# Factral/unsupervised-hyperspectral-nerf

Measured on AMD Instinct MI355X. Metric: train rays/sec (hotdog-shaped 31-band, C2), higher is better.
Workload: dtype f32; 1 GPU; C2 hotdog 31-band rgb+spectral train step (fwd+loss+bwd+Adam); rays_per_gpu=4096, samples_per_ray=64, bands=31, endmembers=6, global_rays=4096, hash_table=16x2^19x2 f32, parallelism=dp1

## Files before the change

### unsupervised-hyperspectral-nerf_amd/csrc/umhs_hashgrid.hip

```cpp
#include <atomic>
#include <cstdlib>

#include "umhs_hashgrid_part.h"

__global__ __launch_bounds__(256) void hashgrid_fwd_kernel(const float* __restrict__ pos01,
                                                           const float2* __restrict__ table,
                                                           const float* __restrict__ scalings, int64_t n, int n_levels,
                                                           int log2_T, float* __restrict__ enc, int64_t stride_n,
                                                           int64_t stride_l) {
  int64_t i = (int64_t)blockIdx.x * 256 + threadIdx.x;
  if (i >= n) return;
  const float px = pos01[3 * i], py = pos01[3 * i + 1], pz = pos01[3 * i + 2];
  const int l = (int)blockIdx.y;
  HashCorners h = hash_corners(px, py, pz, scalings[l], (1u << log2_T) - 1u, (uint32_t)l << log2_T);
  float2 f[8];
  hash_gather8(table, h, f);
  const float2 r = hash_trilerp(f, h.ox, h.oy, h.oz);
  float* o = enc + i * stride_n + (int64_t)l * stride_l;
  if (((stride_n | stride_l) & 1) == 0) {
    *reinterpret_cast<float2*>(o) = r;
  } else {
    o[0] = r.x, o[1] = r.y;
  }
}

extern "C" int umhs_hashgrid_fwd(const float* pos01, const float* table, const float* scalings, int64_t n,
                                 int n_levels, int log2_T, float* enc, int64_t stride_n, int64_t stride_l,
                                 umhs_stream_t stream) {
  if (n < 0 || !table || !scalings) return UMHS_ERR_ARG;
  if (n_levels < 1 || n_levels > 32 || log2_T < 1 || log2_T > 24) return UMHS_ERR_UNSUPPORTED;
  if (n == 0) return UMHS_OK;
  if (!pos01 || !enc) return UMHS_ERR_ARG;
  if (((uintptr_t)table & 15) || ((uintptr_t)enc & 7)) return UMHS_ERR_ARG;
  const float2* t2 = reinterpret_cast<const float2*>(table);
  dim3 grid((unsigned)((n + 255) / 256), (unsigned)n_levels);
  hipLaunchKernelGGL(hashgrid_fwd_kernel, grid, dim3(256), 0, umhs_s(stream), pos01, t2, scalings, n, n_levels, log2_T, enc, stride_n, stride_l);
  UMHS_CHECK_LAUNCH();
  return UMHS_OK;
}

__global__ __launch_bounds__(256) void hashgrid_bwd_kernel(const float* __restrict__ pos01,
                                                           const float* __restrict__ d_enc, int64_t stride_n,
                                                           int64_t stride_l, const float* __restrict__ scalings,
                                                           int64_t n, int log2_T, float* __restrict__ d_table, int level0) {
  int64_t i = (int64_t)blockIdx.x * 256 + threadIdx.x;
  if (i >= n) return;
  int l = level0 + blockIdx.y;
  const float* g = d_enc + i * stride_n + (int64_t)l * stride_l;
  float g0 = g[0], g1 = g[1];
  if (g0 == 0.0f && g1 == 0.0f) return;
  HashCorners h = hash_corners(pos01[3 * i], pos01[3 * i + 1], pos01[3 * i + 2], scalings[l],
                               (1u << log2_T) - 1u, (uint32_t)l << log2_T);
  float ox = h.ox, oy = h.oy, oz = h.oz, rx = 1.0f - ox, ry = 1.0f - oy, rz = 1.0f - oz;
  float w[8];
  w[0] = ox * oy * oz, w[3] = rx * oy * oz, w[1] = ox * ry * oz, w[2] = rx * ry * oz;
  w[4] = ox * oy * rz, w[7] = rx * oy * rz, w[5] = ox * ry * rz, w[6] = rx * ry * rz;
#pragma unroll
  for (int c = 0; c < 8; ++c) {
    if (w[c] != 0.0f) {
      atomicAdd(d_table + 2 * (size_t)h.idx[c], w[c] * g0);
      atomicAdd(d_table + 2 * (size_t)h.idx[c] + 1, w[c] * g1);
    }
  }
}

static_assert(HB_RUN == 512, "hashgrid_fwd_count_kernel's workgroup is one run of the partition");
__global__ __launch_bounds__(HB_RUN) void hashgrid_fwd_count_kernel(const float2* __restrict__ table, float* __restrict__ enc, int64_t stride_n,
                                                                 int64_t stride_l, HbArgs a) {
  __shared__ uint32_t cursor[HB_MAX_NB];
  const int tid = threadIdx.x, lane = tid & 63, wg = blockIdx.x, l = blockIdx.y;
  if (tid < HB_MAX_NB) cursor[tid] = 0;
  __syncthreads();
  const int64_t i = (int64_t)wg * HB_RUN + tid;
  const bool act = i < a.n;
  const int64_t ii = act ? i : a.n - 1;
  const uint32_t mask = (1u << a.log2_T) - 1u, base = (uint32_t)l << a.log2_T;
  const HashCorners h = hash_corners(a.pos01[3 * ii], a.pos01[3 * ii + 1], a.pos01[3 * ii + 2], a.scalings[l], mask, base);
  HashGather hg;
  hash_gather8_issue(table, h, hg);
  __builtin_amdgcn_sched_barrier(0);
  uint32_t slot[8];
#pragma unroll
  for (int c = 0; c < 8; ++c) slot[c] = h.idx[c] - base;
  const uint32_t kx = act ? h.fx : 0xffffffffu, ky = act ? h.fy : 0u, kz = act ? h.fz : 0u;
  const uint32_t kf = act ? (h.eqx | (h.eqy << 1) | (h.eqz << 2)) : (0x80000000u | (uint32_t)lane);
  hb_count_sample(slot, kx, ky, kz, kf, act, a.bucket_bits, lane, cursor);
  __syncthreads();
  if (tid < a.nb) a.wg_counts[((size_t)l * a.nwg + wg) * a.nb + tid] = cursor[tid];
  __builtin_amdgcn_sched_barrier(0);
  float2 f[8];
  hash_gather8_select(h, hg, f);
  const float2 r = hash_trilerp(f, h.ox, h.oy, h.oz);
  if (act) {
    float* o = enc + i * stride_n + (int64_t)l * stride_l;
    if (((stride_n | stride_l) & 1) == 0) {
      *reinterpret_cast<float2*>(o) = r;
    } else {
      o[0] = r.x, o[1] = r.y;
    }
  }
}

static inline int hb_scatter_wgs(int n_levels) {
  static const int forced = [] {
    const char* e = getenv("UMHS_HB_WGS");
    return e ? atoi(e) : 0;
  }();
  int w = forced > 0 ? forced : 1024 / (n_levels > 0 ? n_levels : 1);
  w = (w + 7) / 8 * 8;
  return w < 8 ? 8 : w;
}

struct HbLayout {
  int bucket_bits, nb, nwg;
  size_t cap;
  size_t counts, offsets, lmax, wg_counts, wg_prefix, recs, total;
};

static HbLayout hb_layout(int64_t n, int n_levels, int log2_T) {
  HbLayout w{};
  if (n <= 0 || n_levels < 1 || log2_T < 2) return w;
  w.bucket_bits = log2_T < HB_BUCKET_BITS ? log2_T : HB_BUCKET_BITS, w.nb = 1 << (log2_T - w.bucket_bits);
  if (w.nb > HB_MAX_NB) return w;
  w.nwg = (int)((n + HB_RUN - 1) / HB_RUN);
  w.cap = ((size_t)n * HB_CAP_PER_SAMPLE + 7) & ~(size_t)7;
  if (w.cap >= ((size_t)1 << 28)) return w;
  const auto align = [](size_t x) { return (x + 255) & ~(size_t)255; };
  const size_t m = (size_t)n_levels * w.nb, wg_bytes = align((size_t)n_levels * w.nwg * w.nb * 4);
  w.counts = 0, w.offsets = m * 4, w.lmax = 2 * m * 4;
  w.wg_counts = align((2 * m + (size_t)n_levels * HB_LMAX_PARTS) * 4);
  w.wg_prefix = w.wg_counts + wg_bytes;
  w.recs = w.wg_prefix + wg_bytes;
  w.total = 256 + w.recs + align((size_t)n_levels * w.cap * 16);
  return w;
}

extern "C" size_t umhs_hashgrid_bwd_workspace_bytes(int64_t n, int n_levels, int log2_T) { return hb_layout(n, n_levels, log2_T).total; }

static int hb_args(HbArgs* a, const float* pos01, const float* scalings, int64_t n, int ws_begin, int ws_levels, int log2_T,
                   void* workspace, size_t workspace_bytes) {
  const HbLayout w = hb_layout(n, ws_levels, log2_T);
  if (w.total == 0) return UMHS_ERR_UNSUPPORTED;
  if (!workspace || workspace_bytes < w.total) return UMHS_ERR_WORKSPACE;
  a->pos01 = pos01, a->d_enc = nullptr, a->sn = 0, a->sl = 0, a->scalings = scalings, a->n = n;
  a->log2_T = log2_T, a->bucket_bits = w.bucket_bits, a->nb = w.nb, a->level0 = ws_begin;
  a->nlev = ws_levels, a->lev_off = 0, a->overwrite = 0, a->grad_mask = 0;
  a->adam = HbAdam{};
  a->nwg = w.nwg, a->cap = (uint32_t)w.cap;
  char* const base = reinterpret_cast<char*>(((uintptr_t)workspace + 255) & ~(uintptr_t)255);
  a->counts = reinterpret_cast<uint32_t*>(base + w.counts), a->offsets = reinterpret_cast<uint32_t*>(base + w.offsets);
  a->lmax = reinterpret_cast<uint32_t*>(base + w.lmax);
  a->wg_counts = reinterpret_cast<uint32_t*>(base + w.wg_counts), a->wg_prefix = reinterpret_cast<uint32_t*>(base + w.wg_prefix);
  a->recs = reinterpret_cast<uint4*>(base + w.recs);
  return UMHS_OK;
}

static int hb_run_prepare(const HbArgs& a, int n_levels, int count_wgs, umhs_stream_t stream) {
  if (a.grad_mask && !a.d_enc) return UMHS_ERR_ARG;
  if (n_levels != a.nlev) return UMHS_ERR_ARG;
  dim3 pgrid((unsigned)(count_wgs > 0 && count_wgs < a.nwg ? count_wgs : a.nwg), (unsigned)n_levels);
  hipLaunchKernelGGL(hg_partition_kernel<false>, pgrid, dim3(256), 0, umhs_s(stream), a);
  hipLaunchKernelGGL(hg_wgscan_kernel, dim3((unsigned)a.nb, (unsigned)n_levels), dim3(256), 0, umhs_s(stream), a);
  hipLaunchKernelGGL(hg_scan_kernel, dim3((unsigned)n_levels), dim3(64), 0, umhs_s(stream), a);
  UMHS_CHECK_LAUNCH();
  return UMHS_OK;
}

static int hb_run_apply(const HbArgs& a, int n_levels, float* d_table, umhs_stream_t stream) {
  if (!a.d_enc || !d_table || !a.pos01 || !a.scalings) return UMHS_ERR_ARG;
  int per_level = hb_scatter_wgs(n_levels);
  if (per_level > HB_LMAX_PARTS) per_level = HB_LMAX_PARTS;
  if (per_level > ((a.nwg + 7) / 8) * 8) per_level = ((a.nwg + 7) / 8) * 8;
  dim3 pgrid((unsigned)per_level, (unsigned)n_levels);
  hipLaunchKernelGGL(hg_partition_kernel<true>, pgrid, dim3(256), 0, umhs_s(stream), a);
  const size_t lds = (size_t)(2 << a.bucket_bits) * 8;
  {
    static std::atomic<size_t> granted[16];
    int dev = 0;
    if (hipGetDevice(&dev) != hipSuccess || dev < 0 || dev >= 16) dev = -1;
    if (dev < 0 || granted[dev].load(std::memory_order_relaxed) < lds) {
      if (hipFuncSetAttribute(reinterpret_cast<const void*>(hg_reduce_kernel), hipFuncAttributeMaxDynamicSharedMemorySize,
                              (int)lds) != hipSuccess)
        return UMHS_ERR_LAUNCH;
      if (dev >= 0) granted[dev].store(lds, std::memory_order_relaxed);
    }
  }
  hipLaunchKernelGGL(hg_reduce_kernel, dim3((unsigned)a.nb, (unsigned)n_levels), dim3(1024), lds, umhs_s(stream), a, d_table);
  UMHS_CHECK_LAUNCH();
  return UMHS_OK;
}

extern "C" int umhs_hashgrid_bwd(const float* pos01, const float* d_enc, int64_t stride_n, int64_t stride_l,
                                 const float* scalings, int64_t n, int level_begin, int n_levels, int log2_T,
                                 float* d_table, int overwrite, void* workspace, size_t workspace_bytes,
                                 umhs_stream_t stream) {
  if (n < 0 || !scalings || !d_table || level_begin < 0) return UMHS_ERR_ARG;
  if (n > 0 && (!pos01 || !d_enc)) return UMHS_ERR_ARG;
  if (overwrite && (!workspace || n == 0)) {
    if (hipMemsetAsync(d_table + (((size_t)level_begin << log2_T) * 2), 0, ((size_t)n_levels << log2_T) * 8, umhs_s(stream)) !=
        hipSuccess)
      return UMHS_ERR_LAUNCH;
  }
  if (n_levels < 1 || level_begin + n_levels > 32 || log2_T < 2 || log2_T > 24) return UMHS_ERR_UNSUPPORTED;
  if (n == 0) return UMHS_OK;
  if (!workspace) {
    dim3 grid((unsigned)((n + 255) / 256), (unsigned)n_levels);
    hipLaunchKernelGGL(hashgrid_bwd_kernel, grid, dim3(256), 0, umhs_s(stream), pos01, d_enc, stride_n, stride_l,
                       scalings, n, log2_T, d_table, level_begin);
    UMHS_CHECK_LAUNCH();
    return UMHS_OK;
  }
  HbArgs a;
  int rc = hb_args(&a, pos01, scalings, n, level_begin, n_levels, log2_T, workspace, workspace_bytes);
  if (rc) return rc;
  if ((uintptr_t)d_table & 15) return UMHS_ERR_WORKSPACE;
  a.d_enc = d_enc, a.sn = stride_n, a.sl = stride_l, a.overwrite = overwrite, a.grad_mask = 1;
  rc = hb_run_prepare(a, n_levels, 0, stream);
  if (rc) return rc;
  return hb_run_apply(a, n_levels, d_table, stream);
}

extern "C" int umhs_hashgrid_bwd_prepare(const float* pos01, const float* scalings, int64_t n, int level_begin, int n_levels,
                                         int log2_T, void* workspace, size_t workspace_bytes, umhs_stream_t stream) {
  if (n < 0 || !scalings || level_begin < 0) return UMHS_ERR_ARG;
  if (n_levels < 1 || level_begin + n_levels > 32 || log2_T < 2 || log2_T > 24) return UMHS_ERR_UNSUPPORTED;
  if (n == 0) return UMHS_OK;
  if (!pos01) return UMHS_ERR_ARG;
  HbArgs a;
  int rc = hb_args(&a, pos01, scalings, n, level_begin, n_levels, log2_T, workspace, workspace_bytes);
  if (rc) return rc;
  const int throttle = 16;
  return hb_run_prepare(a, n_levels, throttle, stream);
}

extern "C" int umhs_hashgrid_fwd_count(const float* pos01, const float* table, const float* scalings, int64_t n, int n_levels, int log2_T,
                                       float* enc, int64_t stride_n, int64_t stride_l, void* workspace, size_t workspace_bytes,
                                       umhs_stream_t stream) {
  if (n < 0 || !table || !scalings) return UMHS_ERR_ARG;
  if (n_levels < 1 || n_levels > 32 || log2_T < 2 || log2_T > 24) return UMHS_ERR_UNSUPPORTED;
  if (n == 0) return UMHS_OK;
  if (!pos01 || !enc) return UMHS_ERR_ARG;
  if (((uintptr_t)table & 15) || ((uintptr_t)enc & 7)) return UMHS_ERR_ARG;
  HbArgs a;
  int rc = hb_args(&a, pos01, scalings, n, 0, n_levels, log2_T, workspace, workspace_bytes);
  if (rc) return rc;
  hipLaunchKernelGGL(hashgrid_fwd_count_kernel, dim3((unsigned)a.nwg, (unsigned)n_levels), dim3(HB_RUN), 0, umhs_s(stream),
                     reinterpret_cast<const float2*>(table), enc, stride_n, stride_l, a);
  UMHS_CHECK_LAUNCH();
  return UMHS_OK;
}

extern "C" int umhs_hashgrid_bwd_prepare_counted(const float* pos01, const float* scalings, int64_t n, int n_levels, int log2_T,
                                                 void* workspace, size_t workspace_bytes, umhs_stream_t stream) {
  if (n < 0 || !pos01 || !scalings) return UMHS_ERR_ARG;
  if (n_levels < 1 || n_levels > 32 || log2_T < 2 || log2_T > 24) return UMHS_ERR_UNSUPPORTED;
  if (n == 0) return UMHS_OK;
  HbArgs a;
  int rc = hb_args(&a, pos01, scalings, n, 0, n_levels, log2_T, workspace, workspace_bytes);
  if (rc) return rc;
  hipLaunchKernelGGL(hg_wgscan_kernel, dim3((unsigned)a.nb, (unsigned)n_levels), dim3(256), 0, umhs_s(stream), a);
  hipLaunchKernelGGL(hg_scan_kernel, dim3((unsigned)n_levels), dim3(64), 0, umhs_s(stream), a);
  UMHS_CHECK_LAUNCH();
  return UMHS_OK;
}

static int hb_apply(const float* pos01, const float* d_enc, int64_t stride_n, int64_t stride_l, const float* scalings, int64_t n,
                    int level_begin, int n_levels, int ws_level_begin, int ws_n_levels, int log2_T, float* d_table, int overwrite,
                    const HbAdam* adam, void* workspace, size_t workspace_bytes, umhs_stream_t stream) {
  if (n < 0 || !scalings || !d_table || level_begin < 0) return UMHS_ERR_ARG;
  if (n > 0 && (!pos01 || !d_enc)) return UMHS_ERR_ARG;
  if (n_levels < 1 || level_begin < ws_level_begin || level_begin + n_levels > ws_level_begin + ws_n_levels ||
      ws_level_begin + ws_n_levels > 32 || log2_T < 2 || log2_T > 24)
    return UMHS_ERR_UNSUPPORTED;
  if ((uintptr_t)d_table & 15) return UMHS_ERR_WORKSPACE;
  if (n == 0) {
    if (overwrite && hipMemsetAsync(d_table + (((size_t)level_begin << log2_T) * 2), 0, ((size_t)n_levels << log2_T) * 8,
                                    umhs_s(stream)) != hipSuccess)
      return UMHS_ERR_LAUNCH;
    return UMHS_OK;
  }
  HbArgs a;
  int rc = hb_args(&a, pos01, scalings, n, ws_level_begin, ws_n_levels, log2_T, workspace, workspace_bytes);
  if (rc) return rc;
  a.d_enc = d_enc, a.sn = stride_n, a.sl = stride_l, a.lev_off = level_begin - ws_level_begin, a.overwrite = overwrite;
  if (adam) a.adam = *adam;
  return hb_run_apply(a, n_levels, d_table, stream);
}

extern "C" int umhs_hashgrid_bwd_apply(const float* pos01, const float* d_enc, int64_t stride_n, int64_t stride_l,
                                       const float* scalings, int64_t n, int level_begin, int n_levels, int ws_level_begin,
                                       int ws_n_levels, int log2_T, float* d_table, int overwrite, void* workspace,
                                       size_t workspace_bytes, umhs_stream_t stream) {
  return hb_apply(pos01, d_enc, stride_n, stride_l, scalings, n, level_begin, n_levels, ws_level_begin, ws_n_levels, log2_T, d_table,
                  overwrite, nullptr, workspace, workspace_bytes, stream);
}

extern "C" int umhs_hashgrid_bwd_apply_adam(const float* pos01, const float* d_enc, int64_t stride_n, int64_t stride_l,
                                            const float* scalings, int64_t n, int level_begin, int n_levels, int ws_level_begin,
                                            int ws_n_levels, int log2_T, float* d_table, void* workspace, size_t workspace_bytes,
                                            float* table_params, float* exp_avg, float* exp_avg_sq, float lr, float beta1,
                                            float beta2, float eps, int64_t step, int adam_level_begin, umhs_stream_t stream) {
  if (!table_params || !exp_avg || !exp_avg_sq || step < 1 || adam_level_begin < 0) return UMHS_ERR_ARG;
  if (((uintptr_t)table_params | (uintptr_t)exp_avg | (uintptr_t)exp_avg_sq) & 15) return UMHS_ERR_ARG;
  if (n <= 0) return UMHS_ERR_UNSUPPORTED;
  const AdamBias bc = adam_bias(lr, beta1, beta2, step);
  HbAdam ad;
  ad.p = table_params, ad.m = exp_avg, ad.v = exp_avg_sq, ad.lr_bc1 = bc.lr_bc1, ad.b1 = beta1, ad.b2 = beta2, ad.eps = eps;
  ad.sqrt_bc2 = bc.sqrt_bc2, ad.level_begin = adam_level_begin;
  return hb_apply(pos01, d_enc, stride_n, stride_l, scalings, n, level_begin, n_levels, ws_level_begin, ws_n_levels, log2_T, d_table,
                  1, &ad, workspace, workspace_bytes, stream);
}

__global__ __launch_bounds__(256) void enc_gather_kernel(const float2* __restrict__ in, const int64_t* __restrict__ idx, int64_t m,
                                                         int64_t n, float2* __restrict__ out) {
  const int64_t i = (int64_t)blockIdx.x * 256 + threadIdx.x;
  if (i >= n) return;
  int64_t j = idx[i];
  j = j < 0 ? 0 : (j >= m ? m - 1 : j);
  const int l = blockIdx.y;
  out[(int64_t)l * n + i] = in[(int64_t)l * m + j];
}

extern "C" int umhs_enc_gather(const float* enc_in, const int64_t* index, int64_t m, int64_t n, int n_levels, float* enc_out,
                               umhs_stream_t stream) {
  if (m < 0 || n < 0 || n_levels < 1 || n_levels > 64) return UMHS_ERR_ARG;
  if (n == 0) return UMHS_OK;
  if (m < 1 || !enc_in || !index || !enc_out || (((uintptr_t)enc_in | (uintptr_t)enc_out) & 7)) return UMHS_ERR_ARG;
  hipLaunchKernelGGL(enc_gather_kernel, dim3((unsigned)((n + 255) / 256), (unsigned)n_levels), dim3(256), 0, umhs_s(stream),
                     reinterpret_cast<const float2*>(enc_in), index, m, n, reinterpret_cast<float2*>(enc_out));
  UMHS_CHECK_LAUNCH();
  return UMHS_OK;
}
```

### unsupervised-hyperspectral-nerf_amd/csrc/umhs_hashgrid_part.h

```cpp
#pragma once
#include "umhs_adam.h"
#include "umhs_hash.h"

#define HB_BUCKET_BITS 13
#define HB_MAX_NB 128
#define HB_SPT 2
#define HB_RUN (256 * HB_SPT)
#define HB_CAP_PER_SAMPLE 5
#define HB_MERGE_MIN 16
#define HB_POISON 0xffffffffu
#define HB_LMAX_PARTS 128

struct HbAdam {
  float *p, *m, *v;
  float lr_bc1, b1, b2, eps, sqrt_bc2;
  int level_begin;
};

struct HbArgs {
  HbAdam adam;
  const float* pos01;
  const float* d_enc;
  int64_t sn, sl;
  const float* scalings;
  int64_t n;
  int log2_T, bucket_bits, nb, level0, nlev;
  int lev_off;
  int grad_mask;
  uint32_t *counts, *offsets;
  uint32_t *wg_counts, *wg_prefix;
  int nwg;
  uint32_t* lmax;
  uint4* recs;
  uint32_t cap;
  int overwrite;
};

template <int D>
__device__ __forceinline__ float row_shr(float v) {
  return __int_as_float(__builtin_amdgcn_update_dpp(0, __float_as_int(v), 0x110 + D, 0xF, 0xF, true));
}
template <int D>
__device__ __forceinline__ uint32_t row_shr_u(uint32_t v) {
  return (uint32_t)__builtin_amdgcn_update_dpp(0, (int)v, 0x110 + D, 0xF, 0xF, true);
}
__device__ __forceinline__ int row_shl1(int v) {
  return __builtin_amdgcn_update_dpp(0, v, 0x101, 0xF, 0xF, true);
}
__device__ __forceinline__ uint32_t wave_scan_incl_dpp(uint32_t v) {
  v += row_shr_u<1>(v);
  v += row_shr_u<2>(v);
  v += row_shr_u<4>(v);
  v += row_shr_u<8>(v);
  v += (uint32_t)__builtin_amdgcn_update_dpp(0, (int)v, 0x142, 0xA, 0xF, false);
  v += (uint32_t)__builtin_amdgcn_update_dpp(0, (int)v, 0x143, 0xC, 0xF, false);
  return v;
}
__device__ __forceinline__ uint32_t wave_max_u32_dpp(uint32_t v) {
  v = max(v, row_shr_u<1>(v)), v = max(v, row_shr_u<2>(v)), v = max(v, row_shr_u<4>(v)), v = max(v, row_shr_u<8>(v));
  return max(max((uint32_t)__builtin_amdgcn_readlane((int)v, 15), (uint32_t)__builtin_amdgcn_readlane((int)v, 31)),
             max((uint32_t)__builtin_amdgcn_readlane((int)v, 47), (uint32_t)__builtin_amdgcn_readlane((int)v, 63)));
}
template <int D>
__device__ __forceinline__ void seg_scan_step(float2 (&val)[8], bool& f, int l16) {
  const bool take = l16 >= D && !f;
#pragma unroll
  for (int c = 0; c < 8; ++c) {
    const float px = row_shr<D>(val[c].x), py = row_shr<D>(val[c].y);
    if (take) val[c].x += px, val[c].y += py;
  }
  const int pf = (int)row_shr_u<D>((uint32_t)f);
  if (l16 >= D) f = f || pf;
}

#ifdef UMHS_HG_STAMP
__device__ unsigned long long g_hg_stamp[2][16][16];
#define HG_STAMP_DECL unsigned long long hgs_acc_[15] = {}, hgs_t_ = hg_now_(false)
__device__ __forceinline__ unsigned long long hg_now_(bool drain) {
  unsigned long long t;
  __builtin_amdgcn_sched_barrier(0);
  if (drain) {
    asm volatile("s_waitcnt vmcnt(0)\n\ts_memtime %0\n\ts_waitcnt lgkmcnt(0)" : "=s"(t)::"memory");
  } else {
    asm volatile("s_memtime %0\n\ts_waitcnt lgkmcnt(0)" : "=s"(t)::"memory");
  }
  __builtin_amdgcn_sched_barrier(0);
  return t;
}
#define HG_STAMP(k_)                              \
  do {                                            \
    const unsigned long long n_ = hg_now_(false); \
    hgs_acc_[k_] += n_ - hgs_t_, hgs_t_ = n_;     \
  } while (0)
#define HG_STAMP_DRAIN(k_)                       \
  do {                                           \
    const unsigned long long n_ = hg_now_(true); \
    hgs_acc_[k_] += n_ - hgs_t_, hgs_t_ = n_;    \
  } while (0)
#define HG_STAMP_FLUSH(kern_, lev_)                                                                                     \
  do {                                                                                                                  \
    if ((threadIdx.x & 63) == 0) {                                                                                      \
      _Pragma("unroll") for (int q_ = 0; q_ < 15; ++q_) if (hgs_acc_[q_]) atomicAdd(&g_hg_stamp[kern_][(lev_) & 15][q_], hgs_acc_[q_]); \
      atomicAdd(&g_hg_stamp[kern_][(lev_) & 15][15], 1ull);                                                             \
    }                                                                                                                   \
  } while (0)
extern "C" int umhs_debug_hg_stamps(unsigned long long* out) {
  return (int)hipMemcpyFromSymbol(out, HIP_SYMBOL(g_hg_stamp), sizeof(unsigned long long) * 2 * 16 * 16);
}
extern "C" int umhs_debug_hg_stamps_clear() {
  static unsigned long long z[2 * 16 * 16] = {};
  return (int)hipMemcpyToSymbol(HIP_SYMBOL(g_hg_stamp), z, sizeof(z));
}
#else
#define HG_STAMP_DECL \
  do {                \
  } while (0)
#define HG_STAMP(k_) \
  do {               \
  } while (0)
#define HG_STAMP_DRAIN(k_) \
  do {                     \
  } while (0)
#define HG_STAMP_FLUSH(kern_, lev_) \
  do {                              \
  } while (0)
#endif


struct HbIn {
  float g[HB_SPT][2], p[HB_SPT][3];
  uint32_t c[2], mb[2];
};

template <bool SCATTER>
__device__ __forceinline__ void hb_load(const HbArgs& a, const int wg, const int lev, const int l, HbIn& in) {
  const int tid = threadIdx.x;
#pragma unroll
  for (int k = 0; k < HB_SPT; ++k) {
    const int64_t i = (int64_t)wg * HB_RUN + k * 256 + tid, ii = i < a.n ? i : a.n - 1;
    in.g[k][0] = in.g[k][1] = 0.0f;
    if (SCATTER || a.grad_mask) {
      const float* g = a.d_enc + ii * a.sn + (int64_t)l * a.sl;
      if (((a.sn | a.sl) & 1) == 0 && (((uintptr_t)a.d_enc) & 7) == 0) {
        const float2 g2 = *reinterpret_cast<const float2*>(g);
        in.g[k][0] = g2.x, in.g[k][1] = g2.y;
      } else {
        in.g[k][0] = g[0], in.g[k][1] = g[1];
      }
    }
    in.p[k][0] = a.pos01[3 * ii], in.p[k][1] = a.pos01[3 * ii + 1], in.p[k][2] = a.pos01[3 * ii + 2];
  }
  in.c[0] = in.c[1] = in.mb[0] = in.mb[1] = 0u;
  if (SCATTER && tid < 64) {
#pragma unroll
    for (int h = 0; h < 2; ++h) {
      const int bk = tid + 64 * h;
      if (bk < a.nb) {
        const size_t o = ((size_t)lev * a.nwg + wg) * a.nb + bk;
        in.c[h] = a.wg_counts[o];
        in.mb[h] = a.offsets[lev * a.nb + bk] + a.wg_prefix[o];
      }
    }
  }
}

template <bool SCATTER>
__device__ __forceinline__ void hg_partition_body(const HbArgs& a, const int wg, const int lev, const int l, const float s, const HbIn& in,
                                                  uint32_t& wgmax) {
  __shared__ uint32_t cursor[HB_MAX_NB];
  __shared__ uint32_t delta[HB_MAX_NB];
  __shared__ uint32_t ltotal;
  constexpr int MAXREC = SCATTER ? HB_RUN * 4 : 1;
  __shared__ uint4 stage[MAXREC];
  const int tid = threadIdx.x, lane = tid & 63;
  HG_STAMP_DECL;
  if (!SCATTER && tid < HB_MAX_NB) cursor[tid] = 0;
  if (SCATTER && tid < 64) {
    uint32_t carry = 0;
#pragma unroll
    for (int h = 0; h < 2; ++h) {
      const int bk = tid + 64 * h;
      const uint32_t c = in.c[h], mb = in.mb[h];
      const uint32_t incl = wave_scan_incl_dpp(c);
      const uint32_t first = carry + incl - c;
      carry += (uint32_t)__builtin_amdgcn_readlane((int)incl, 63);
      cursor[bk] = first, delta[bk] = mb - first;
    }
    if (tid == 0) ltotal = carry;
  }
  __syncthreads();
  const uint32_t mask = (1u << a.log2_T) - 1u;
  const int bb = a.bucket_bits;
  uint4* const __restrict__ out = a.recs + (size_t)lev * a.cap;
  const bool staged = SCATTER && ltotal <= (uint32_t)MAXREC;
  if (SCATTER) HG_STAMP_DRAIN(0);
  uint32_t vmax = 0u;
  auto emit = [&](const uint32_t meta, const float vx, const float vy, const float ox) {
    const uint32_t b = __builtin_amdgcn_ubfe(meta, (uint32_t)bb, (uint32_t)(24 - bb));
    const uint32_t pos = atomicAdd(&cursor[b], 1u);
    if (!SCATTER) return;
    const uint4 r = make_uint4(__float_as_uint(vx), __float_as_uint(vy), __float_as_uint(ox), meta);
    if (staged)
      stage[pos] = r;
    else
      out[delta[b] + pos] = r;
  };
#pragma unroll
  for (int k = 0; k < HB_SPT; ++k) {
    const int64_t i = (int64_t)wg * HB_RUN + k * 256 + tid;
    bool act = false;
    float g0 = 0.0f, g1 = 0.0f, ox = 0.0f, oy = 0.0f, oz = 0.0f;
    uint32_t kx = 0xffffffffu, ky = 0, kz = 0, kf = 0x80000000u | (uint32_t)lane;
    uint32_t slot[8];
#pragma unroll
    for (int c = 0; c < 8; ++c) slot[c] = 0;
    if (SCATTER) HG_STAMP_DRAIN(1);
    if (i < a.n) {
      g0 = in.g[k][0], g1 = in.g[k][1];
      if (!a.grad_mask || g0 != 0.0f || g1 != 0.0f) {
        act = true;
        HashCorners h = hash_corners(in.p[k][0], in.p[k][1], in.p[k][2], s, mask, 0u);
        ox = h.ox, oy = h.oy, oz = h.oz;
#pragma unroll
        for (int c = 0; c < 8; ++c) slot[c] = h.idx[c];
        kx = h.fx, ky = h.fy, kz = h.fz, kf = h.eqx | (h.eqy << 1) | (h.eqz << 2);
      }
    }
    if (SCATTER) HG_STAMP(2);
    const int l16 = lane & 15;
    const uint32_t px_ = row_shr_u<1>(kx), py_ = row_shr_u<1>(ky), pz_ = row_shr_u<1>(kz), pf_ = row_shr_u<1>(kf);
    bool head = (l16 == 0) | (px_ != kx) | (py_ != ky) | (pz_ != kz) | (pf_ != kf);
    const bool merging = __builtin_popcountll(__builtin_amdgcn_ballot_w64(!head)) >= HB_MERGE_MIN;
    if (!merging) head = true;
    const int nhead = merging ? row_shl1((int)head) : 1;
    const bool tail = act && (l16 == 15 || nhead);
    const bool solo = head && tail;
    const float rx = 1.0f - ox, ry = 1.0f - oy, rz = 1.0f - oz;
    float2 val[8];
    if (SCATTER && merging) {
      float w[8];
      w[0] = ox * oy * oz, w[3] = rx * oy * oz, w[1] = ox * ry * oz, w[2] = rx * ry * oz;
      w[4] = ox * oy * rz, w[7] = rx * oy * rz, w[5] = ox * ry * rz, w[6] = rx * ry * rz;
#pragma unroll
      for (int c = 0; c < 8; ++c) val[c] = act ? make_float2(w[c] * g0, w[c] * g1) : make_float2(0.0f, 0.0f);
      bool f = head;
      seg_scan_step<1>(val, f, l16), seg_scan_step<2>(val, f, l16);
      seg_scan_step<4>(val, f, l16), seg_scan_step<8>(val, f, l16);
    }
    if (SCATTER) HG_STAMP(3);
    if (tail) {
      const uint32_t single = 15u << 24;
      if (solo) {
        const uint32_t pm = slot[HASH_FI[0]] ^ slot[HASH_CI[0]];
        const float wyz[4] = {oy * oz, ry * oz, oy * rz, ry * rz};
        if (SCATTER) vmax = max(vmax, max(__float_as_uint(fabsf(g0)), __float_as_uint(fabsf(g1))));
        if ((pm >> bb) == 0) {
          const uint32_t km = (pm ? (uint32_t)(31 - __clz((int)pm)) : 15u) << 24;
          uint32_t meta[4], pos[4], bk[4];
#pragma unroll
          for (int p = 0; p < 4; ++p) {
            meta[p] = slot[HASH_FI[p]] | km;
            bk[p] = __builtin_amdgcn_ubfe(meta[p], (uint32_t)bb, (uint32_t)(24 - bb));
            pos[p] = atomicAdd(&cursor[bk[p]], 1u);
          }
          if (SCATTER) {
#pragma unroll
            for (int p = 0; p < 4; ++p) {
              const uint4 r = make_uint4(__float_as_uint(g0 * wyz[p]), __float_as_uint(g1 * wyz[p]), __float_as_uint(ox), meta[p]);
              if (staged)
                stage[pos[p]] = r;
              else
                out[delta[bk[p]] + pos[p]] = r;
            }
          }
        } else {
#pragma unroll
          for (int p = 0; p < 4; ++p) {
            const float gx = g0 * wyz[p], gy = g1 * wyz[p];
            emit(slot[HASH_FI[p]] | single, gx * rx, gy * rx, 0.0f);
            emit(slot[HASH_CI[p]] | single, gx * ox, gy * ox, 0.0f);
          }
        }
      } else {
#pragma unroll
        for (int c = 0; c < 8; ++c) {
          if (SCATTER) vmax = max(vmax, max(__float_as_uint(fabsf(val[c].x)), __float_as_uint(fabsf(val[c].y))));
          emit(slot[c] | single, SCATTER ? val[c].x : 0.0f, SCATTER ? val[c].y : 0.0f, 0.0f);
        }
      }
    }
    if (SCATTER) HG_STAMP(4);
  }
  if (!SCATTER) {
    __syncthreads();
    if (tid < a.nb) a.wg_counts[((size_t)lev * a.nwg + wg) * a.nb + tid] = cursor[tid];
    return;
  }
  vmax = wave_max_u32_dpp(vmax);
  if (lane == 0 && vmax > 0u) atomicMax(&wgmax, vmax);
  HG_STAMP(5);
  __syncthreads();
  HG_STAMP(6);
  if (staged) {
    char* const ob = reinterpret_cast<char*>(out);
    const uint32_t total = ltotal;
    for (uint32_t i = tid; i < total; i += 256) {
      const uint4 r = stage[i];
      const uint32_t b = __builtin_amdgcn_ubfe(r.w, (uint32_t)bb, (uint32_t)(24 - bb));
      *reinterpret_cast<uint4*>(ob + (size_t)((delta[b] + i) << 4)) = r;
    }
  }
  HG_STAMP_DRAIN(7);
  HG_STAMP_FLUSH(0, l);
}

__device__ __forceinline__ void hb_count_sample(const uint32_t (&slot)[8], const uint32_t kx, const uint32_t ky, const uint32_t kz, const uint32_t kf,
                                                const bool act, const int bb, const int lane, uint32_t* __restrict__ cursor) {
  const int l16 = lane & 15;
  const uint32_t px_ = row_shr_u<1>(kx), py_ = row_shr_u<1>(ky), pz_ = row_shr_u<1>(kz), pf_ = row_shr_u<1>(kf);
  bool head = (l16 == 0) | (px_ != kx) | (py_ != ky) | (pz_ != kz) | (pf_ != kf);
  const bool merging = __builtin_popcountll(__builtin_amdgcn_ballot_w64(!head)) >= HB_MERGE_MIN;
  if (!merging) head = true;
  const int nhead = merging ? row_shl1((int)head) : 1;
  const bool tail = act && (l16 == 15 || nhead);
  const bool solo = head && tail;
  if (tail) {
    if (solo) {
      const uint32_t pm = slot[3] ^ slot[0];
      static_assert(HASH_FI[0] == 3 && HASH_FI[1] == 2 && HASH_FI[2] == 7 && HASH_FI[3] == 6 && HASH_CI[0] == 0, "corner order");
      atomicAdd(&cursor[slot[3] >> bb], 1u), atomicAdd(&cursor[slot[2] >> bb], 1u);
      atomicAdd(&cursor[slot[7] >> bb], 1u), atomicAdd(&cursor[slot[6] >> bb], 1u);
      if ((pm >> bb) != 0) {
        atomicAdd(&cursor[slot[0] >> bb], 1u), atomicAdd(&cursor[slot[1] >> bb], 1u);
        atomicAdd(&cursor[slot[4] >> bb], 1u), atomicAdd(&cursor[slot[5] >> bb], 1u);
      }
    } else {
      atomicAdd(&cursor[slot[0] >> bb], 1u), atomicAdd(&cursor[slot[1] >> bb], 1u);
      atomicAdd(&cursor[slot[2] >> bb], 1u), atomicAdd(&cursor[slot[3] >> bb], 1u);
      atomicAdd(&cursor[slot[4] >> bb], 1u), atomicAdd(&cursor[slot[5] >> bb], 1u);
      atomicAdd(&cursor[slot[6] >> bb], 1u), atomicAdd(&cursor[slot[7] >> bb], 1u);
    }
  }
}

template <bool SCATTER>
__global__ __launch_bounds__(256) void hg_partition_kernel(HbArgs a) {
  const int lev = a.lev_off + blockIdx.y, l = a.level0 + lev;
  const float s = a.scalings[l];
  __shared__ uint32_t wgmax;
  HbIn cur;
  if (threadIdx.x == 0) wgmax = 0;
  if (SCATTER) {
    const int per = (a.nwg + 7) >> 3, q = (int)(gridDim.x >> 3);
    const int x = (int)(blockIdx.x & 7u), end = min(a.nwg, (x + 1) * per);
    int wg = x * per + (int)(blockIdx.x >> 3);
    const uint32_t lmax0 = a.lmax[(size_t)lev * HB_LMAX_PARTS];
    if (wg >= end) return;
    hb_load<true>(a, wg, lev, l, cur);
    if (lmax0 == HB_POISON) return;
    while (true) {
      const int nxt = wg + q;
      HbIn nx;
      if (nxt < end) hb_load<true>(a, nxt, lev, l, nx);
      hg_partition_body<true>(a, wg, lev, l, s, cur, wgmax);
      if (nxt >= end) break;
      cur = nx, wg = nxt;
      __syncthreads();
    }
    __syncthreads();
    if (threadIdx.x == 0 && wgmax) a.lmax[(size_t)lev * HB_LMAX_PARTS + (blockIdx.x % HB_LMAX_PARTS)] = wgmax;
  } else {
    for (int wg = blockIdx.x; wg < a.nwg; wg += gridDim.x) {
      hb_load<false>(a, wg, lev, l, cur);
      hg_partition_body<false>(a, wg, lev, l, s, cur, wgmax);
      __syncthreads();
    }
  }
}

__global__ __launch_bounds__(256) void hg_wgscan_kernel(HbArgs a) {
  __shared__ uint32_t wsum[4];
  const int tid = threadIdx.x, lane = tid & 63, wv = tid >> 6, b = blockIdx.x, lev = blockIdx.y;
  const int per = (a.nwg + 255) / 256, w0 = min(a.nwg, tid * per), w1 = min(a.nwg, w0 + per);
  const uint32_t* __restrict__ col = a.wg_counts + (size_t)lev * a.nwg * a.nb + b;
  uint32_t* __restrict__ pre = a.wg_prefix + (size_t)lev * a.nwg * a.nb + b;
  uint32_t sum = 0;
  for (int w = w0; w < w1; ++w) sum += col[(size_t)w * a.nb];
  uint32_t incl = sum;
#pragma unroll
  for (int d = 1; d < 64; d <<= 1) {
    const uint32_t o = __shfl_up(incl, d, 64);
    if (lane >= d) incl += o;
  }
  if (lane == 63) wsum[wv] = incl;
  __syncthreads();
  uint32_t run = incl - sum, total = 0;
#pragma unroll
  for (int k = 0; k < 4; ++k) {
    if (k < wv) run += wsum[k];
    total += wsum[k];
  }
  for (int w = w0; w < w1; ++w) {
    pre[(size_t)w * a.nb] = run;
    run += col[(size_t)w * a.nb];
  }
  if (tid == 0) a.counts[lev * a.nb + b] = total;
}

__global__ void hg_scan_kernel(HbArgs a) {
  const int lane = threadIdx.x, lev = blockIdx.x;
  uint32_t carry = 0;
  for (int b0 = 0; b0 < a.nb; b0 += 64) {
    const int b = b0 + lane;
    const uint32_t c = b < a.nb ? a.counts[lev * a.nb + b] : 0u;
    uint32_t incl = c;
#pragma unroll
    for (int d = 1; d < 64; d <<= 1) {
      const uint32_t o = __shfl_up(incl, d, 64);
      if (lane >= d) incl += o;
    }
    if (b < a.nb) a.offsets[lev * a.nb + b] = carry + incl - c;
    carry += __shfl(incl, 63, 64);
  }
  for (int j = lane; j < HB_LMAX_PARTS; j += 64) a.lmax[(size_t)lev * HB_LMAX_PARTS + j] = (j == 0 && carry > a.cap) ? HB_POISON : 0u;
}

__device__ __forceinline__ unsigned long long hb_fixed(const float x) {
  const float fl = floorf(x);
  const int hi = (int)fl;
  const uint32_t lo = (uint32_t)((x - fl) * 4294967296.0f);
  return ((unsigned long long)(uint32_t)hi << 32) | lo;
}

__global__ __launch_bounds__(1024) void hg_reduce_kernel(HbArgs a, float* __restrict__ d_table) {
  extern __shared__ __attribute__((aligned(16))) long long tile[];
  const int tid = threadIdx.x, b = blockIdx.x, lev = a.lev_off + blockIdx.y, l = a.level0 + lev;
  HG_STAMP_DECL;
  const uint32_t start = a.offsets[lev * a.nb + b], cnt = a.counts[lev * a.nb + b];
  const int nsl = 2 << a.bucket_bits;
  const size_t slab = 2 * (((size_t)l << a.log2_T) + ((size_t)b << a.bucket_bits));
  const bool adam = a.adam.p != nullptr && l >= a.adam.level_begin;
  auto step4 = [&](const float4& g, float4& pp, float4& mm, float4& vv) {
    adam_update(pp.x, mm.x, vv.x, g.x, a.adam.lr_bc1, a.adam.b1, a.adam.b2, a.adam.eps, a.adam.sqrt_bc2);
    adam_update(pp.y, mm.y, vv.y, g.y, a.adam.lr_bc1, a.adam.b1, a.adam.b2, a.adam.eps, a.adam.sqrt_bc2);
    adam_update(pp.z, mm.z, vv.z, g.z, a.adam.lr_bc1, a.adam.b1, a.adam.b2, a.adam.eps, a.adam.sqrt_bc2);
    adam_update(pp.w, mm.w, vv.w, g.w, a.adam.lr_bc1, a.adam.b1, a.adam.b2, a.adam.eps, a.adam.sqrt_bc2);
  };
  const uint32_t lmax_bits =
      wave_max_u32_dpp(max(a.lmax[(size_t)lev * HB_LMAX_PARTS + (tid & 63)], a.lmax[(size_t)lev * HB_LMAX_PARTS + 64 + (tid & 63)]));
  const bool nan_level = lmax_bits >= 0x7f800000u && (cnt != 0 || lmax_bits == HB_POISON);
  const bool from_tile = cnt != 0 && !nan_level;
  if (!from_tile && !a.overwrite && !nan_level) return;
  int kfix = 0;
  if (from_tile) {
    for (int i = tid; i < nsl; i += 1024) tile[i] = 0;
    int e;
    (void)frexpf(__uint_as_float(lmax_bits), &e);
    const int hb = 33 - __clz(cnt);
    kfix = min(62 - hb - e, 150);
    __syncthreads();
    const uint4* __restrict__ rp = a.recs + (size_t)lev * a.cap + start;
    typedef unsigned long long u64;
    u64* ut = reinterpret_cast<u64*>(tile);
    const uint32_t lowmask = (1u << a.bucket_bits) - 1u;
    const float fscale = ldexpf(1.0f, kfix - 32);
    auto add = [&](const uint4& r) {
      const float vx = __uint_as_float(r.x), vy = __uint_as_float(r.y), ox = __uint_as_float(r.z);
      const uint32_t s = r.w & lowmask, kk = (r.w >> 24) & 15u;
      const float rx = (1.0f - ox) * fscale, oxs = ox * fscale;
      atomicAdd(&ut[2 * s], hb_fixed(vx * rx)), atomicAdd(&ut[2 * s + 1], hb_fixed(vy * rx));
      if (kk != 15u) {
        const uint32_t cs = s ^ (((2u << kk) - 1u) & lowmask);
        atomicAdd(&ut[2 * cs], hb_fixed(vx * oxs)), atomicAdd(&ut[2 * cs + 1], hb_fixed(vy * oxs));
      }
    };
    uint32_t i = tid;
    HG_STAMP(0);
    const uint32_t last = cnt - 1;
    auto load4 = [&](uint4 (&r)[4], const uint32_t at) {
#pragma unroll
      for (int u = 0; u < 4; ++u) r[u] = rp[min(at + 1024u * u, last)];
    };
    auto add4 = [&](const uint4 (&r)[4], const uint32_t at) {
      add(r[0]);
#pragma unroll
      for (int u = 1; u < 4; ++u)
        if (at + 1024u * u < cnt) add(r[u]);
    };
    uint4 ra[4], rb[4];
    if (i < cnt) {
      load4(ra, i);
      while (true) {
        HG_STAMP_DRAIN(1);
        load4(rb, i + 4096u);
        add4(ra, i);
        HG_STAMP(3);
        i += 4096u;
        if (i >= cnt) break;
        HG_STAMP_DRAIN(1);
        load4(ra, i + 4096u);
        add4(rb, i);
        HG_STAMP(3);
        i += 4096u;
        if (i >= cnt) break;
      }
    }
    HG_STAMP_DRAIN(3);
    __syncthreads();
    HG_STAMP(4);
  }
  float* const dst = d_table + slab;
  const float qnan = __uint_as_float(0x7fc00000u);
  for (int j0 = tid * 4; j0 < nsl; j0 += 4 * 4096) {
    float4 pp[4], mm[4], vv[4], dd[4];
#pragma unroll
    for (int c = 0; c < 4; ++c) {
      const int j = min(j0 + c * 4096, nsl - 4);
      if (adam) {
        pp[c] = *reinterpret_cast<const float4*>(a.adam.p + slab + j), mm[c] = *reinterpret_cast<const float4*>(a.adam.m + slab + j);
        vv[c] = *reinterpret_cast<const float4*>(a.adam.v + slab + j);
      }
      if (!a.overwrite) dd[c] = *reinterpret_cast<const float4*>(dst + j);
    }
#pragma unroll
    for (int c = 0; c < 4; ++c) {
      const int j = j0 + c * 4096;
      if (j < nsl) {
        float4 d = a.overwrite ? make_float4(0.f, 0.f, 0.f, 0.f) : dd[c];
        if (nan_level) {
          d = make_float4(qnan, qnan, qnan, qnan);
        } else if (from_tile) {
          d.x += (float)ldexp((double)tile[j], -kfix), d.y += (float)ldexp((double)tile[j + 1], -kfix);
          d.z += (float)ldexp((double)tile[j + 2], -kfix), d.w += (float)ldexp((double)tile[j + 3], -kfix);
        }
        *reinterpret_cast<float4*>(dst + j) = d;
        if (adam) {
          step4(d, pp[c], mm[c], vv[c]);
          *reinterpret_cast<float4*>(a.adam.p + slab + j) = pp[c];
          *reinterpret_cast<float4*>(a.adam.m + slab + j) = mm[c];
          *reinterpret_cast<float4*>(a.adam.v + slab + j) = vv[c];
        }
      }
    }
  }
  HG_STAMP_DRAIN(5);
  HG_STAMP_FLUSH(1, l);
}
```

Measured before the change: 6.010 million rays/s.

## Make hashgrid reduce kernel persistent with cross-tile prefetch of records and headers

Result: no change. 5.960 million rays/s (-0.8%).

```diff
diff --git a/unsupervised-hyperspectral-nerf_amd/csrc/umhs_hashgrid.hip b/unsupervised-hyperspectral-nerf_amd/csrc/umhs_hashgrid.hip
--- a/unsupervised-hyperspectral-nerf_amd/csrc/umhs_hashgrid.hip
+++ b/unsupervised-hyperspectral-nerf_amd/csrc/umhs_hashgrid.hip
@@ -174,18 +174,37 @@
   dim3 pgrid((unsigned)per_level, (unsigned)n_levels);
   hipLaunchKernelGGL(hg_partition_kernel<true>, pgrid, dim3(256), 0, umhs_s(stream), a);
   const size_t lds = (size_t)(2 << a.bucket_bits) * 8;
+  int cus = 0;
   {
     static std::atomic<size_t> granted[16];
+    static std::atomic<int> cu_count[16];
     int dev = 0;
     if (hipGetDevice(&dev) != hipSuccess || dev < 0 || dev >= 16) dev = -1;
     if (dev < 0 || granted[dev].load(std::memory_order_relaxed) < lds) {
-      if (hipFuncSetAttribute(reinterpret_cast<const void*>(hg_reduce_kernel), hipFuncAttributeMaxDynamicSharedMemorySize,
+      if (hipFuncSetAttribute(reinterpret_cast<const void*>(hg_reduce_kernel<true>), hipFuncAttributeMaxDynamicSharedMemorySize,
+                              (int)lds) != hipSuccess ||
+          hipFuncSetAttribute(reinterpret_cast<const void*>(hg_reduce_kernel<false>), hipFuncAttributeMaxDynamicSharedMemorySize,
                               (int)lds) != hipSuccess)
         return UMHS_ERR_LAUNCH;
       if (dev >= 0) granted[dev].store(lds, std::memory_order_relaxed);
     }
-  }
-  hipLaunchKernelGGL(hg_reduce_kernel, dim3((unsigned)a.nb, (unsigned)n_levels), dim3(1024), lds, umhs_s(stream), a, d_table);
+    if (dev >= 0) cus = cu_count[dev].load(std::memory_order_relaxed);
+    if (cus <= 0) {
+      int cur = dev;
+      if ((cur < 0 && hipGetDevice(&cur) != hipSuccess) || hipDeviceGetAttribute(&cus, hipDeviceAttributeMultiprocessorCount, cur) != hipSuccess ||
+          cus <= 0)
+        return UMHS_ERR_LAUNCH;
+      if (dev >= 0) cu_count[dev].store(cus, std::memory_order_relaxed);
+    }
+  }
+  const int tiles = a.nb * n_levels;
+  int wgs = cus;
+  if (const char* e = getenv("UMHS_HR_WGS"); e && *e) wgs = atoi(e) < 1 ? 1 : atoi(e);
+  if (wgs > tiles) wgs = tiles;
+  if (a.bucket_bits == HB_BUCKET_BITS)
+    hipLaunchKernelGGL(hg_reduce_kernel<true>, dim3((unsigned)wgs), dim3(1024), lds, umhs_s(stream), a, d_table, tiles);
+  else
+    hipLaunchKernelGGL(hg_reduce_kernel<false>, dim3((unsigned)wgs), dim3(1024), lds, umhs_s(stream), a, d_table, tiles);
   UMHS_CHECK_LAUNCH();
   return UMHS_OK;
 }
diff --git a/unsupervised-hyperspectral-nerf_amd/csrc/umhs_hashgrid_part.h b/unsupervised-hyperspectral-nerf_amd/csrc/umhs_hashgrid_part.h
--- a/unsupervised-hyperspectral-nerf_amd/csrc/umhs_hashgrid_part.h
+++ b/unsupervised-hyperspectral-nerf_amd/csrc/umhs_hashgrid_part.h
@@ -104,6 +104,10 @@
       atomicAdd(&g_hg_stamp[kern_][(lev_) & 15][15], 1ull);                                                             \
     }                                                                                                                   \
   } while (0)
+#define HG_STAMP_RESET                                                   \
+  do {                                                                   \
+    _Pragma("unroll") for (int q_ = 0; q_ < 15; ++q_) hgs_acc_[q_] = 0; \
+  } while (0)
 extern "C" int umhs_debug_hg_stamps(unsigned long long* out) {
   return (int)hipMemcpyFromSymbol(out, HIP_SYMBOL(g_hg_stamp), sizeof(unsigned long long) * 2 * 16 * 16);
 }
@@ -123,6 +127,9 @@
   } while (0)
 #define HG_STAMP_FLUSH(kern_, lev_) \
   do {                              \
+  } while (0)
+#define HG_STAMP_RESET \
+  do {                 \
   } while (0)
 #endif
 
@@ -432,117 +439,182 @@
   return ((unsigned long long)(uint32_t)hi << 32) | lo;
 }
 
-__global__ __launch_bounds__(1024) void hg_reduce_kernel(HbArgs a, float* __restrict__ d_table) {
+#define HG_READ4(r_) asm volatile("" ::"v"((r_)[0]), "v"((r_)[1]), "v"((r_)[2]), "v"((r_)[3]))
+typedef uint32_t hb_rec __attribute__((ext_vector_type(4)));
+template <bool FULL>
+__global__ __launch_bounds__(1024) void hg_reduce_kernel(HbArgs a, float* __restrict__ d_table, const int tiles) {
   extern __shared__ __attribute__((aligned(16))) long long tile[];
-  const int tid = threadIdx.x, b = blockIdx.x, lev = a.lev_off + blockIdx.y, l = a.level0 + lev;
+  typedef unsigned long long u64;
+  const int tid = threadIdx.x, lane = tid & 63, G = (int)gridDim.x;
+  const int nsl = FULL ? (2 << HB_BUCKET_BITS) : (2 << a.bucket_bits), nbs = a.log2_T - a.bucket_bits;
+  const uint32_t lowmask = FULL ? (1u << HB_BUCKET_BITS) - 1u : (1u << a.bucket_bits) - 1u;
+  const float qnan = __uint_as_float(0x7fc00000u);
+  u64* const ut = reinterpret_cast<u64*>(tile);
   HG_STAMP_DECL;
-  const uint32_t start = a.offsets[lev * a.nb + b], cnt = a.counts[lev * a.nb + b];
-  const int nsl = 2 << a.bucket_bits;
-  const size_t slab = 2 * (((size_t)l << a.log2_T) + ((size_t)b << a.bucket_bits));
-  const bool adam = a.adam.p != nullptr && l >= a.adam.level_begin;
   auto step4 = [&](const float4& g, float4& pp, float4& mm, float4& vv) {
     adam_update(pp.x, mm.x, vv.x, g.x, a.adam.lr_bc1, a.adam.b1, a.adam.b2, a.adam.eps, a.adam.sqrt_bc2);
     adam_update(pp.y, mm.y, vv.y, g.y, a.adam.lr_bc1, a.adam.b1, a.adam.b2, a.adam.eps, a.adam.sqrt_bc2);
     adam_update(pp.z, mm.z, vv.z, g.z, a.adam.lr_bc1, a.adam.b1, a.adam.b2, a.adam.eps, a.adam.sqrt_bc2);
     adam_update(pp.w, mm.w, vv.w, g.w, a.adam.lr_bc1, a.adam.b1, a.adam.b2, a.adam.eps, a.adam.sqrt_bc2);
   };
-  const uint32_t lmax_bits =
-      wave_max_u32_dpp(max(a.lmax[(size_t)lev * HB_LMAX_PARTS + (tid & 63)], a.lmax[(size_t)lev * HB_LMAX_PARTS + 64 + (tid & 63)]));
-  const bool nan_level = lmax_bits >= 0x7f800000u && (cnt != 0 || lmax_bits == HB_POISON);
-  const bool from_tile = cnt != 0 && !nan_level;
-  if (!from_tile && !a.overwrite && !nan_level) return;
-  int kfix = 0;
-  if (from_tile) {
-    for (int i = tid; i < nsl; i += 1024) tile[i] = 0;
-    int e;
-    (void)frexpf(__uint_as_float(lmax_bits), &e);
-    const int hb = 33 - __clz(cnt);
-    kfix = min(62 - hb - e, 150);
-    __syncthreads();
-    const uint4* __restrict__ rp = a.recs + (size_t)lev * a.cap + start;
-    typedef unsigned long long u64;
-    u64* ut = reinterpret_cast<u64*>(tile);
-    const uint32_t lowmask = (1u << a.bucket_bits) - 1u;
-    const float fscale = ldexpf(1.0f, kfix - 32);
-    auto add = [&](const uint4& r) {
-      const float vx = __uint_as_float(r.x), vy = __uint_as_float(r.y), ox = __uint_as_float(r.z);
-      const uint32_t s = r.w & lowmask, kk = (r.w >> 24) & 15u;
-      const float rx = (1.0f - ox) * fscale, oxs = ox * fscale;
-      atomicAdd(&ut[2 * s], hb_fixed(vx * rx)), atomicAdd(&ut[2 * s + 1], hb_fixed(vy * rx));
-      if (kk != 15u) {
-        const uint32_t cs = s ^ (((2u << kk) - 1u) & lowmask);
-        atomicAdd(&ut[2 * cs], hb_fixed(vx * oxs)), atomicAdd(&ut[2 * cs + 1], hb_fixed(vy * oxs));
-      }
+  const uint32_t* const hbase = (lane & 1) ? a.counts : a.offsets;
+  auto head_load = [&](const int tt, const int have, uint32_t& hv, uint32_t& m0, uint32_t& m1) {
+    const int lv = a.lev_off + (tt >> nbs);
+    hv = hbase[lv * a.nb + (tt & (a.nb - 1))];
+    if (lv != have) m0 = a.lmax[(size_t)lv * HB_LMAX_PARTS + lane], m1 = a.lmax[(size_t)lv * HB_LMAX_PARTS + 64 + lane];
+    return lv;
+  };
+  auto head_start = [](const uint32_t hv) { return (uint32_t)__builtin_amdgcn_readlane((int)hv, 0); };
+  auto head_count = [](const uint32_t hv) { return (uint32_t)__builtin_amdgcn_readlane((int)hv, 1); };
+  auto is_nan_level = [](const uint32_t lmax_bits, const uint32_t cn) { return lmax_bits >= 0x7f800000u && (cn != 0 || lmax_bits == HB_POISON); };
+  auto load4 = [&](hb_rec (&r)[4], const uint4* __restrict__ rp, const uint32_t at, const uint32_t cn) {
+#pragma unroll
+    for (int u = 0; u < 4; ++u) r[u] = *reinterpret_cast<const hb_rec*>(reinterpret_cast<const char*>(rp) + (min(at + 1024u * u, cn - 1) << 4));
+  };
+  auto ld4 = [](const float* base, const uint32_t byte_off) { return *reinterpret_cast<const float4*>(reinterpret_cast<const char*>(base) + byte_off); };
+  auto st4 = [](float* base, const uint32_t byte_off, const float4& v) { *reinterpret_cast<float4*>(reinterpret_cast<char*>(base) + byte_off) = v; };
+  hb_rec ra[4], rb[4];
+  int t = blockIdx.x;
+  uint32_t hv, lm0 = 0u, lm1 = 0u;
+  int lev = head_load(t, -1, hv, lm0, lm1);
+  for (int i = tid; i < nsl; i += 1024) tile[i] = 0;
+  uint32_t start = head_start(hv), cnt = head_count(hv);
+  uint32_t lmax_bits = wave_max_u32_dpp(max(lm0, lm1));
+  bool nan_level = is_nan_level(lmax_bits, cnt), from_tile = cnt != 0 && !nan_level;
+  if (from_tile) load4(ra, a.recs + (size_t)lev * a.cap + start, (uint32_t)tid, cnt);
+  __syncthreads();
+  while (true) {
+    const int tn = t + G;
+    const bool more = tn < tiles;
+    int nlev = lev;
+    if (more) nlev = head_load(tn, lev, hv, lm0, lm1);
+    const int l = a.level0 + lev, b = t & (a.nb - 1);
+    int j0 = tid * 4;
+    uint32_t rt = tid;
+    asm volatile("" : "+v"(j0), "+v"(rt));
+    const auto live = [&](const int c) { return FULL || j0 + c * 4096 < nsl; };
+    const auto coff = [&](const int c) { return 4u * (uint32_t)(FULL ? j0 + c * 4096 : min(j0 + c * 4096, nsl - 4)); };
+    const size_t slab = 2 * (((size_t)l << a.log2_T) + ((size_t)b << a.bucket_bits));
+    const bool adam = a.adam.p != nullptr && a.overwrite && l >= a.adam.level_begin;
+    const bool work = from_tile || a.overwrite || nan_level;
+    float* const dst = d_table + slab;
+    float4 q[6];
+    if (work) {
+      if (adam) {
+#pragma unroll
+        for (int c = 0; c < 2; ++c) q[3 * c] = ld4(a.adam.p + slab, coff(c)), q[3 * c + 1] = ld4(a.adam.m + slab, coff(c)), q[3 * c + 2] = ld4(a.adam.v + slab, coff(c));
+      } else if (!a.overwrite) {
+#pragma unroll
+        for (int c = 0; c < 4; ++c) q[c] = ld4(dst, coff(c));
+      }
+    }
+    HG_STAMP(0);
+    float4 gf[4];
+    if (from_tile) {
+      int e;
+      (void)frexpf(__uint_as_float(lmax_bits), &e);
+      const int hb = 33 - __clz(cnt);
+      const int kfix = min(62 - hb - e, 150);
+      const uint4* __restrict__ rp = a.recs + (size_t)lev * a.cap + start;
+      const float fscale = ldexpf(1.0f, kfix - 32);
+      auto add = [&](const hb_rec& r) {
+        const float vx = __uint_as_float(r.x), vy = __uint_as_float(r.y), ox = __uint_as_float(r.z);
+        const uint32_t s = r.w & lowmask, kk = (r.w >> 24) & 15u;
+        const float rx = (1.0f - ox) * fscale, oxs = ox * fscale;
+        atomicAdd(&ut[2 * s], hb_fixed(vx * rx)), atomicAdd(&ut[2 * s + 1], hb_fixed(vy * rx));
+        if (kk != 15u) {
+          const uint32_t cs = s ^ (((2u << kk) - 1u) & lowmask);
+          atomicAdd(&ut[2 * cs], hb_fixed(vx * oxs)), atomicAdd(&ut[2 * cs + 1], hb_fixed(vy * oxs));
+        }
+      };
+      auto add4 = [&](const hb_rec (&r)[4], const uint32_t at) {
+#pragma unroll
+        for (int u = 0; u < 4; ++u) {
+          asm volatile("" ::"v"(r[u]));
+          if (at + 1024u * u < cnt) add(r[u]);
+        }
+      };
+      uint32_t base = 0;
+      while (base + 4096u < cnt) {
+        HG_STAMP_DRAIN(1);
+        load4(rb, rp, base + 4096u + rt, cnt);
+        add4(ra, base + rt);
+        HG_STAMP(3);
+        HG_STAMP_DRAIN(1);
+        load4(ra, rp, base + 8192u + rt, cnt);
+        add4(rb, base + 4096u + rt);
+        HG_STAMP(3);
+        base += 8192u;
+      }
+      HG_STAMP_DRAIN(1);
+      if (base < cnt) add4(ra, base + rt);
+      HG_STAMP_DRAIN(3);
+      __syncthreads();
+#pragma unroll
+      for (int c = 0; c < 4; ++c) {
+        const int j = j0 + c * 4096;
+        if (live(c)) {
+          gf[c].x = (float)ldexp((double)tile[j], -kfix), gf[c].y = (float)ldexp((double)tile[j + 1], -kfix);
+          gf[c].z = (float)ldexp((double)tile[j + 2], -kfix), gf[c].w = (float)ldexp((double)tile[j + 3], -kfix);
+          tile[j] = 0, tile[j + 1] = 0, tile[j + 2] = 0, tile[j + 3] = 0;
+        }
+      }
+      __syncthreads();
+      HG_STAMP(4);
+    } else {
+#pragma unroll
+      for (int c = 0; c < 4; ++c) gf[c] = nan_level ? make_float4(qnan, qnan, qnan, qnan) : make_float4(0.f, 0.f, 0.f, 0.f);
+    }
+    HG_READ4(ra);
+    HG_READ4(rb);
+    asm volatile("" ::"v"(q[0].x), "v"(q[1].x), "v"(q[2].x), "v"(q[3].x), "v"(q[4].x), "v"(q[5].x), "v"(hv), "v"(lm0), "v"(lm1));
+    asm volatile("" : "+v"(j0), "+v"(rt));
+    uint32_t nlmax_bits = lmax_bits;
+    bool nnan = false, nfrom = false;
+    uint32_t nstart = 0u, ncnt = 0u;
+    if (more) {
+      nstart = head_start(hv), ncnt = head_count(hv);
+      const uint32_t level_max = wave_max_u32_dpp(max(lm0, lm1));
+      if (nlev != lev) nlmax_bits = level_max;
+      nnan = is_nan_level(nlmax_bits, ncnt), nfrom = ncnt != 0 && !nnan;
+      if (nfrom) load4(ra, a.recs + (size_t)nlev * a.cap + nstart, rt, ncnt);
+    }
+    auto grad4 = [&](const int c, float4 d) {
+      if (nan_level) {
+        d = gf[c];
+      } else if (from_tile) {
+        d.x += gf[c].x, d.y += gf[c].y, d.z += gf[c].z, d.w += gf[c].w;
+      }
+      return d;
     };
-    uint32_t i = tid;
-    HG_STAMP(0);
-    const uint32_t last = cnt - 1;
-    auto load4 = [&](uint4 (&r)[4], const uint32_t at) {
-#pragma unroll
-      for (int u = 0; u < 4; ++u) r[u] = rp[min(at + 1024u * u, last)];
-    };
-    auto add4 = [&](const uint4 (&r)[4], const uint32_t at) {
-      add(r[0]);
-#pragma unroll
-      for (int u = 1; u < 4; ++u)
-        if (at + 1024u * u < cnt) add(r[u]);
-    };
-    uint4 ra[4], rb[4];
-    if (i < cnt) {
-      load4(ra, i);
-      while (true) {
-        HG_STAMP_DRAIN(1);
-        load4(rb, i + 4096u);
-        add4(ra, i);
-        HG_STAMP(3);
-        i += 4096u;
-        if (i >= cnt) break;
-        HG_STAMP_DRAIN(1);
-        load4(ra, i + 4096u);
-        add4(rb, i);
-        HG_STAMP(3);
-        i += 4096u;
-        if (i >= cnt) break;
-      }
-    }
-    HG_STAMP_DRAIN(3);
-    __syncthreads();
-    HG_STAMP(4);
-  }
-  float* const dst = d_table + slab;
-  const float qnan = __uint_as_float(0x7fc00000u);
-  for (int j0 = tid * 4; j0 < nsl; j0 += 4 * 4096) {
-    float4 pp[4], mm[4], vv[4], dd[4];
-#pragma unroll
-    for (int c = 0; c < 4; ++c) {
-      const int j = min(j0 + c * 4096, nsl - 4);
-      if (adam) {
-        pp[c] = *reinterpret_cast<const float4*>(a.adam.p + slab + j), mm[c] = *reinterpret_cast<const float4*>(a.adam.m + slab + j);
-        vv[c] = *reinterpret_cast<const float4*>(a.adam.v + slab + j);
-      }
-      if (!a.overwrite) dd[c] = *reinterpret_cast<const float4*>(dst + j);
-    }
-#pragma unroll
-    for (int c = 0; c < 4; ++c) {
-      const int j = j0 + c * 4096;
-      if (j < nsl) {
-        float4 d = a.overwrite ? make_float4(0.f, 0.f, 0.f, 0.f) : dd[c];
-        if (nan_level) {
-          d = make_float4(qnan, qnan, qnan, qnan);
-        } else if (from_tile) {
-          d.x += (float)ldexp((double)tile[j], -kfix), d.y += (float)ldexp((double)tile[j + 1], -kfix);
-          d.z += (float)ldexp((double)tile[j + 2], -kfix), d.w += (float)ldexp((double)tile[j + 3], -kfix);
+    if (work && adam) {
+#pragma unroll
+      for (int c = 0; c < 4; ++c) {
+        float4* const pmv = &q[3 * (c & 1)];
+        __builtin_amdgcn_sched_barrier(0);
+        asm volatile("" ::"v"(pmv[0].x), "v"(pmv[1].x), "v"(pmv[2].x));
+        if (live(c)) {
+          const float4 d = grad4(c, make_float4(0.f, 0.f, 0.f, 0.f));
+          st4(dst, coff(c), d);
+          step4(d, pmv[0], pmv[1], pmv[2]);
+          st4(a.adam.p + slab, coff(c), pmv[0]), st4(a.adam.m + slab, coff(c), pmv[1]), st4(a.adam.v + slab, coff(c), pmv[2]);
         }
-        *reinterpret_cast<float4*>(dst + j) = d;
-        if (adam) {
-          step4(d, pp[c], mm[c], vv[c]);
-          *reinterpret_cast<float4*>(a.adam.p + slab + j) = pp[c];
-          *reinterpret_cast<float4*>(a.adam.m + slab + j) = mm[c];
-          *reinterpret_cast<float4*>(a.adam.v + slab + j) = vv[c];
+        if (c < 2) pmv[0] = ld4(a.adam.p + slab, coff(c + 2)), pmv[1] = ld4(a.adam.m + slab, coff(c + 2)), pmv[2] = ld4(a.adam.v + slab, coff(c + 2));
+      }
+      asm volatile("" ::: "memory");
+    } else if (work) {
+#pragma unroll
+      for (int c = 0; c < 4; ++c) {
+        if (live(c)) {
+          st4(dst, coff(c), grad4(c, a.overwrite ? make_float4(0.f, 0.f, 0.f, 0.f) : q[c]));
         }
       }
-    }
-  }
-  HG_STAMP_DRAIN(5);
-  HG_STAMP_FLUSH(1, l);
-}
+      asm volatile("" ::: "memory");
+    }
+    HG_STAMP_DRAIN(5);
+    HG_STAMP_FLUSH(1, l);
+    HG_STAMP_RESET;
+    if (!more) break;
+    t = tn, lev = nlev, start = nstart, cnt = ncnt, lmax_bits = nlmax_bits, nan_level = nnan, from_tile = nfrom;
+  }
+}
```
